# V2AI/EFG

Hardware: AMD Instinct MI355X
Metric: scenes/sec ConQueR 1-frame Waymo train step (higher is better)
Workload: dtype f32; 1 GPU; ConQueR res18 p3, 1-sweep Waymo-shaped scenes, 180000 pts/scene, 0.1 m voxels, 2 scenes/GPU, 900 queries, fwd+bwd+AdamW+OneCycle, graph of `value`: FPN levels / heads the reference evaluates and never reads are skipped (same losses and gradients; the line's `full_graph` object times the full reference graph); global_batch=2, parallelism=dp1

## Files before the change

### efg_amd/_lib.py

```python
import ctypes
import os

import torch

_LIB_PATH = os.path.join(os.path.dirname(os.path.abspath(__file__)), "lib", "libefg_hip.so")
_lib = None

c_void_p, c_int, c_int64, c_size_t, c_float = (ctypes.c_void_p, ctypes.c_int, ctypes.c_int64, ctypes.c_size_t,
                                               ctypes.c_float)

_SIGS = {
    "efg_last_error": (ctypes.c_char_p, []),
    "efg_version": (ctypes.c_char_p, []),
    "efg_capture_stream_create": (ctypes.c_int, [ctypes.POINTER(ctypes.c_void_p)]),
    "efg_capture_stream_destroy": (ctypes.c_int, [ctypes.c_void_p]),
    "efg_dynamic_voxelize_f32": (c_int, [c_void_p, c_int64, c_int, c_void_p, c_void_p, c_void_p, c_void_p]),
    "efg_hard_voxelize_workspace_bytes": (c_size_t, [c_int64, c_int, c_int, c_int, c_int, c_void_p, c_void_p]),
    "efg_hard_voxelize_f32": (c_int, [c_void_p, c_void_p, c_int, c_int, c_void_p, c_void_p, c_int, c_int, c_void_p,
                                      c_void_p, c_int, c_void_p, c_void_p, c_void_p, c_void_p, c_size_t, c_void_p]),
    "efg_hard_voxelize_debug_timeline": (c_size_t, [c_void_p]),
    "efg_scatter_workspace_bytes": (c_size_t, [c_int64, c_int, c_void_p]),
    "efg_scatter_index": (c_int, [c_void_p, c_int64, c_int, c_void_p, c_void_p, c_void_p, c_void_p, c_size_t,
                                  c_void_p]),
    "efg_scatter_reduce_workspace_bytes": (c_size_t, [c_int64, c_int]),
# ... 49 lines not shown
    "efg_box_attn_fused_backward_strided_f32": (c_int, [c_void_p] * 5 + [c_int, c_void_p, c_int, c_void_p, c_void_p] + [c_int] * 8 + [c_void_p] * 4 + [c_size_t, c_void_p]),
    "efg_box_attn_fused_backward_workspace_bytes": (c_size_t, [c_int] * 6),
    "efg_box_attn_fused_backward_f32": (c_int, [c_void_p] * 8 + [c_int] * 8 + [c_void_p] * 4 + [c_size_t, c_void_p]),
    "efg_boxes_bev_f32": (c_int, [c_void_p, c_int, c_void_p, c_int, c_int, c_void_p, c_void_p]),
    "efg_nms_workspace_bytes": (c_size_t, [c_int]),
    "efg_topk_unsorted_f32": (c_int, [c_void_p, c_int64, c_int, c_int, c_void_p, c_void_p, c_void_p]),
    "efg_box_refine_forward_f32": (c_int, [c_void_p, c_void_p, c_int64, c_float, c_void_p, c_void_p]),
    "efg_box_refine_backward_f32": (c_int, [c_void_p, c_void_p, c_void_p, c_int64, c_float, c_void_p, c_void_p, c_void_p]),
    "efg_add_layernorm_forward_f32": (c_int, [c_void_p] * 4 + [c_float, c_int64, c_int] + [c_void_p] * 5),
    "efg_add_layernorm_backward_workspace_bytes": (c_size_t, [c_int64, c_int]),
    "efg_add_layernorm_backward_f32": (c_int, [c_void_p] * 5 + [c_int64, c_int] + [c_void_p] * 4 + [c_size_t, c_void_p]),
    "efg_points_transform_filter_workspace_bytes": (c_size_t, [c_int64]),
    "efg_points_transform_filter_f32": (c_int, [c_void_p, c_int64, c_int, c_void_p, c_int, c_void_p, c_void_p, c_void_p,
                                                c_void_p, c_size_t, c_void_p]),
    "efg_points_gather_f32": (c_int, [c_void_p, c_void_p, c_int64, c_int, c_void_p, c_void_p]),
    "efg_match_cost_f32": (c_int, [c_void_p] * 4 + [c_int] * 5 + [c_float] * 6 + [c_void_p] * 3),
    "efg_focal_loss_forward_f32": (c_int, [c_void_p, c_void_p, c_int, c_int64, c_int, c_float, c_float, c_void_p, c_void_p,
                                           c_void_p]),
    "efg_focal_loss_backward_f32": (c_int, [c_void_p, c_void_p, c_int, c_int64, c_int, c_float, c_float, c_void_p,
                                            c_void_p, c_void_p, c_void_p]),
    "efg_box_loss_forward_f32": (c_int, [c_void_p] * 6 + [c_int64] + [c_int] * 4 + [c_void_p] * 4),
    "efg_box_loss_backward_f32": (c_int, [c_void_p] * 6 + [c_int64] + [c_int] * 4 + [c_void_p] * 5),
    "efg_rot_giou_paired_forward_f32": (c_int, [c_void_p, c_void_p, c_int64] + [c_void_p] * 4),
    "efg_rot_giou_paired_backward_f32": (c_int, [c_void_p, c_void_p, c_int64] + [c_void_p] * 5),
    "efg_bn_workspace_bytes": (c_size_t, [c_int]),
    "efg_bn_forward_f32": (c_int, [c_void_p] * 7 + [c_float, c_float, c_int64, c_int, c_int] + [c_void_p] * 4 +
                           [c_size_t, c_void_p]),
    "efg_bn_backward_f32": (c_int, [c_void_p] * 6 + [c_int64, c_int, c_int] + [c_void_p] * 5 + [c_size_t, c_void_p]),
    "efg_lsap_f32": (c_int, [c_void_p, c_int, c_int, c_int, c_void_p, c_void_p, c_void_p, c_void_p]),
    "efg_nms_f32": (c_int, [c_void_p, c_int, c_float, c_int, c_void_p, c_void_p, c_void_p, c_size_t, c_void_p]),
    "efg_spconv_tile_shape": (c_int, [c_int, c_int, c_int, c_int64, c_int64, c_void_p, c_void_p, c_void_p]),
    "efg_cylinder_select_f32": (c_int, [c_void_p, c_int64, c_int, c_int, c_float, c_void_p, c_void_p, c_int64, c_void_p,
                                        c_void_p, c_void_p, c_int, c_void_p, c_void_p]),
    "efg_attention_fwd_f32": (c_int, [c_void_p, c_int64, c_int64, c_void_p, c_void_p, c_int64, c_int64, c_int64, c_int, c_int,
                                      c_int, c_float, c_void_p, c_void_p, c_void_p]),
    "efg_attention_bwd_f32": (c_int, [c_void_p, c_int64, c_int64, c_void_p, c_void_p, c_int64, c_int64, c_void_p, c_void_p,
                                      c_void_p, c_int64, c_int, c_int, c_int, c_float, c_void_p, c_void_p, c_void_p,
                                      c_void_p]),
    "efg_attention_long_fwd_f32": (c_int, [c_void_p, c_int64, c_int64] * 3 + [c_void_p, c_int, c_int64, c_int, c_int, c_float,
                                                                             c_void_p, c_void_p, c_void_p]),
    "efg_attention_long_bwd_f32": (c_int, [c_void_p, c_int64, c_int64] * 3 + [c_void_p, c_int, c_void_p, c_void_p, c_void_p,
                                                                             c_int64, c_int, c_int, c_float, c_void_p, c_void_p,
                                                                             c_void_p, c_void_p, c_void_p]),
    "efg_relu_bwd_colsum_f32": (c_int, [c_void_p, c_void_p, c_int64, c_int, c_void_p, c_void_p, c_void_p, c_size_t, c_void_p]),
    "efg_nms_segmented_f32": (c_int, [c_void_p, c_void_p, c_int, c_float, c_int, c_void_p, c_void_p, c_void_p, c_size_t,
                                      c_void_p]),
    "efg_gn_workspace_bytes": (c_size_t, [c_int, c_int]),
    "efg_gn_forward_f32": (c_int, [c_void_p] * 3 + [c_float, c_int, c_int64, c_int, c_int] + [c_void_p] * 4 +
                           [c_size_t, c_void_p]),
    "efg_gn_backward_f32": (c_int, [c_void_p] * 5 + [c_int, c_int64, c_int, c_int] + [c_void_p] * 4 +
                            [c_size_t, c_void_p]),
    "efg_colsum_workspace_bytes": (c_size_t, [c_int64, c_int]),
    "efg_colsum_f32": (c_int, [c_void_p, c_int64, c_int, c_int64, c_void_p, c_void_p, c_size_t, c_void_p]),
    "efg_det_eval_max_pred": (c_int, []),
    "efg_det_eval_max_gt": (c_int, []),
    "efg_det_eval_pair_weights_f32": (c_int, [c_void_p] * 7 + [c_int] * 3 + [c_float] * 3 + [c_void_p, c_void_p]),
    "efg_det_eval_assign_f32": (c_int, [c_void_p] * 5 + [c_int] * 3 + [c_void_p] * 7),
    "efg_det_eval_accumulate": (c_int, [c_void_p, c_void_p, c_void_p, c_int] + [c_void_p] * 3),
    "efg_track_eval_mot_f32": (c_int, [c_void_p] * 6 + [c_int] * 4 + [c_void_p] * 5 + [c_int, c_void_p, c_int] +
                               [c_void_p] * 3),
    "efg_track_eval_accumulate": (c_int, [c_void_p, c_void_p, c_void_p, c_int, c_int] + [c_void_p] * 3),
    "efg_nusc_eval_max_gt": (c_int, []),
    "efg_nusc_eval_match_f32": (c_int, [c_void_p] * 3 + [c_int, c_int, c_int64, c_int64] + [c_float] * 4 +
                                [c_void_p, c_void_p]),
    "efg_nusc_eval_errors_f32": (c_int, [c_void_p] * 6 + [c_int64, c_int64, c_int] + [c_void_p] * 3),
    "efg_center_decode_max_cells": (c_int, []),
    "efg_center_decode_max_tasks": (c_int, []),
    "efg_center_decode_candidates_f32": (c_int, [c_void_p, c_void_p] + [c_int] * 4 + [c_float] * 6 + [c_void_p] * 6),
    "efg_circle_nms_f32": (c_int, [c_void_p] * 3 + [c_int, c_int, c_void_p, c_int, c_int] + [c_void_p] * 3),
    "efg_center_decode_boxes_f32": (c_int, [c_void_p, c_void_p] + [c_int] * 5 + [c_void_p] * 10),
    "efg_pillar_workspace_bytes": (c_size_t, []),
    "efg_pillar_forward_f32": (c_int, [c_void_p] * 9 + [c_float, c_float, c_int64] + [c_int] * 4 + [c_float] * 4 + [c_int] +
                               [c_void_p] * 5 + [c_size_t, c_int, c_void_p]),
    "efg_pillar_backward_f32": (c_int, [c_void_p] * 10 + [c_int64] + [c_int] * 4 + [c_float] * 4 + [c_int] + [c_void_p] * 4 +
                                [c_size_t, c_int, c_void_p]),
    "efg_pillar_scatter_f32": (c_int, [c_void_p, c_void_p, c_int64] + [c_int] * 4 + [c_void_p, c_void_p]),
    "efg_pillar_gather_f32": (c_int, [c_void_p, c_void_p, c_int64] + [c_int] * 4 + [c_void_p, c_void_p]),
}

_GEMM_SPLIT_SIGS = {
    "_pack_bytes": (c_size_t, [c_int, c_int]),
    "_pack_f32": (c_int, [c_void_p, c_int64, c_int64, c_int, c_int, c_void_p, c_void_p]),
    "_pack_linear_f32": (c_int, [c_void_p, c_int, c_int, c_void_p, c_void_p, c_void_p]),
    "_f32": (c_int, [c_void_p, c_int64, c_int, c_int64, c_void_p, c_int, c_void_p, c_int, c_void_p, c_int64, c_void_p]),
    "_wgrad_workspace_bytes": (c_size_t, [c_int64, c_int, c_int]),
    "_wgrad_f32": (c_int, [c_void_p, c_int64, c_void_p, c_int64, c_int64, c_int, c_int, c_void_p, c_void_p, c_size_t,
                           c_void_p]),
}
for _prefix in ("efg_gemm_bf16x3", "efg_gemm_bf16x6"):
    _SIGS.update({_prefix + _name: _sig for _name, _sig in _GEMM_SPLIT_SIGS.items()})

EXPORTED_SYMBOLS = tuple(_SIGS)


def lib_path():
    return _LIB_PATH


def _warn_if_stale():
    csrc = os.path.join(os.path.dirname(os.path.abspath(__file__)), "csrc")
    try:
        built = os.path.getmtime(_LIB_PATH)
        newer = [f for f in os.listdir(csrc) if os.path.getmtime(os.path.join(csrc, f)) > built + 1.0]
    except OSError:
        return
    if newer:
# ... 68 lines not shown
```

### efg_amd/build.py

```python
import os
import subprocess
import sys

_PKG = os.path.dirname(os.path.abspath(__file__))
_ROOT = os.path.dirname(_PKG)
CSRC = os.path.join(_PKG, "csrc")
LIB_DIR = os.path.join(_PKG, "lib")
LIB_PATH = os.path.join(LIB_DIR, "libefg_hip.so")

SOURCES = ["lib.cpp", "voxelize.hip", "voxelize_bins.hip", "voxelize_hash.hip", "scatter.hip", "spconv_index.hip", "spconv_conv.hip", "spconv_tiles.hip", "spconv_wgt.hip", "msda.hip", "box_fused.hip", "iou3d_nms.hip", "matcher.hip", "layernorm.hip", "augment.hip", "det_loss.hip", "rot_giou.hip", "batchnorm.hip", "colsum.hip", "crop.hip", "attention.hip", "gemm_bf16x3.hip", "gemm_bf16x6.hip", "topk.hip", "det_eval.hip", "track_eval.hip", "nusc_eval.hip", "center_decode.hip", "pillars.hip"]
FLAGS = ["--offload-arch=gfx950", "-O3", "-std=c++17", "-fPIC", "-munsafe-fp-atomics", "-ffp-contract=off",
         "-Wall", "-Wno-unused-function", "-I" + os.path.join(_ROOT, "include"), "-I" + CSRC]


def _stale(target, deps):
    if not os.path.exists(target):
        return True
    t = os.path.getmtime(target)
    return any(os.path.getmtime(d) > t for d in deps)


def build(force=False, verbose=False):
    os.makedirs(LIB_DIR, exist_ok=True)
    hipcc = os.environ.get("HIPCC", "/opt/rocm/bin/hipcc")
    headers = [os.path.join(CSRC, h) for h in os.listdir(CSRC) if h.endswith(".h")]
    headers.append(os.path.join(_ROOT, "include", "efg_hip.h"))
    objs = []
    procs = []
    for src in SOURCES:
        path = os.path.join(CSRC, src)
        if not os.path.exists(path):
            continue
        obj = os.path.join(LIB_DIR, os.path.splitext(src)[0] + ".o")
        objs.append(obj)
        if force or _stale(obj, [path] + headers):
            cmd = [hipcc] + FLAGS + ["-x", "hip", "-c", path, "-o", obj]
            if verbose:
                print(" ".join(cmd))
            procs.append((src, subprocess.Popen(cmd, stdout=subprocess.PIPE, stderr=subprocess.STDOUT)))
    for src, p in procs:
        out, _ = p.communicate()
        if p.returncode != 0:
            raise RuntimeError("hipcc failed on %s:\n%s" % (src, out.decode()))
        if verbose and out:
            print(out.decode())
    if force or procs or _stale(LIB_PATH, objs):
        cmd = [hipcc, "--offload-arch=gfx950", "-shared", "-fPIC", "-o", LIB_PATH] + objs
        subprocess.check_call(cmd)
    return LIB_PATH


if __name__ == "__main__":
    print(build(force="--force" in sys.argv, verbose=True))
```

### efg_amd/detection3d/utils.py

```python
import copy

import torch
import torch.nn.functional as F
from torch import nn

from ..operators.linear import Linear, linear


class MLP(nn.Module):

    def __init__(self, input_dim, hidden_dim, output_dim, num_layers):
        super().__init__()
        self.num_layers = num_layers
        h = [hidden_dim] * (num_layers - 1)
        self.layers = nn.ModuleList(Linear(n, k) for n, k in zip([input_dim] + h, h + [output_dim]))

    def forward(self, x):
        for i, layer in enumerate(self.layers):
            x = linear(x, layer.weight, layer.bias, relu=True) if i < self.num_layers - 1 else layer(x)
        return x


def get_clones(module, n):
    return nn.ModuleList([copy.deepcopy(module) for _ in range(n)])


def inverse_sigmoid(x, eps=1e-5):
    x = x.clamp(min=0, max=1)
    return torch.log(x.clamp(min=eps) / (1 - x).clamp(min=eps))


def box_cxcyczlwh_to_xyxyxy(x):
    c, s = x[..., :3], x[..., 3:6]
    return torch.cat((c - 0.5 * s, c + 0.5 * s), dim=-1)


def generalized_box3d_iou(boxes1, boxes2):
    boxes1 = torch.nan_to_num(boxes1)
    boxes2 = torch.nan_to_num(boxes2)
    vol1 = (boxes1[:, 3] - boxes1[:, 0]) * (boxes1[:, 4] - boxes1[:, 1]) * (boxes1[:, 5] - boxes1[:, 2])
    vol2 = (boxes2[:, 3] - boxes2[:, 0]) * (boxes2[:, 4] - boxes2[:, 1]) * (boxes2[:, 5] - boxes2[:, 2])
    lo = torch.max(boxes1[:, None, :3], boxes2[:, :3])
    hi = torch.min(boxes1[:, None, 3:], boxes2[:, 3:])
    lwh = (hi - lo).clamp(min=0)
    inter = lwh[:, :, 0] * lwh[:, :, 1] * lwh[:, :, 2]
    union = vol1[:, None] + vol2 - inter
    iou = inter / union
    lo = torch.min(boxes1[:, None, :3], boxes2[:, :3])
    hi = torch.max(boxes1[:, None, 3:], boxes2[:, 3:])
    whl = (hi - lo).clamp(min=0)
    vol = whl[:, :, 0] * whl[:, :, 1] * whl[:, :, 2]
    return iou - (vol - union) / vol


def pairwise_box3d_giou(boxes1, boxes2):
    boxes1 = torch.nan_to_num(boxes1)[..., :, None, :]
    boxes2 = torch.nan_to_num(boxes2)[..., None, :, :]
    vol1 = (boxes1[..., 3] - boxes1[..., 0]) * (boxes1[..., 4] - boxes1[..., 1]) * (boxes1[..., 5] - boxes1[..., 2])
    vol2 = (boxes2[..., 3] - boxes2[..., 0]) * (boxes2[..., 4] - boxes2[..., 1]) * (boxes2[..., 5] - boxes2[..., 2])
    lwh = (torch.min(boxes1[..., 3:], boxes2[..., 3:]) - torch.max(boxes1[..., :3], boxes2[..., :3])).clamp(min=0)
    inter = lwh[..., 0] * lwh[..., 1] * lwh[..., 2]
    union = vol1 + vol2 - inter
    whl = (torch.max(boxes1[..., 3:], boxes2[..., 3:]) - torch.min(boxes1[..., :3], boxes2[..., :3])).clamp(min=0)
    vol = whl[..., 0] * whl[..., 1] * whl[..., 2]
    return inter / union - (vol - union) / vol


def paired_box3d_giou(boxes1, boxes2):
    boxes1 = torch.nan_to_num(boxes1)
    boxes2 = torch.nan_to_num(boxes2)
    vol1 = (boxes1[:, 3] - boxes1[:, 0]) * (boxes1[:, 4] - boxes1[:, 1]) * (boxes1[:, 5] - boxes1[:, 2])
    vol2 = (boxes2[:, 3] - boxes2[:, 0]) * (boxes2[:, 4] - boxes2[:, 1]) * (boxes2[:, 5] - boxes2[:, 2])
# ... 119 lines not shown
```

### efg_amd/operators/linear.py

```python
import importlib
import os

import torch
import torch.nn.functional as F
from torch import nn
from torch.autograd import Function
from torch.autograd.function import once_differentiable

from .. import _lib as L


def column_sum(x2, out=None):
    L.require_gpu(x2)
    if x2.stride(1) != 1:
        x2 = x2.contiguous()
    rows, cols = x2.shape
    if out is None:
        out = torch.empty(cols, dtype=torch.float32, device=x2.device)
    ws_bytes = L.lib().efg_colsum_workspace_bytes(rows, cols)
    ws = torch.empty(max(ws_bytes, 16), dtype=torch.uint8, device=x2.device)
    L.check(L.lib().efg_colsum_f32(x2.data_ptr(), rows, cols, x2.stride(0) if rows > 1 else cols, L.ptr(out), L.ptr(ws),
                                   ws_bytes, L.stream()))
    return out

# ... 54 lines not shown
    if k >= _SPLIT_MIN_ROWS and k % _SPLITS == 0 and x2.is_contiguous() and g2.is_contiguous():
        gs = g2.view(_SPLITS, k // _SPLITS, g2.shape[1])
        xs = x2.view(_SPLITS, k // _SPLITS, x2.shape[1])
        return torch.bmm(gs.transpose(1, 2), xs).sum(0)
    if _WGRAD_ROWMAJOR:
        return g2.t().mm(x2)
    return x2.t().mm(g2).t()


class LinearFunction(Function):
    @staticmethod
    def forward(ctx, x, weight, bias, relu=False):
        x2 = x.reshape(-1, x.shape[-1])
        ctx.packed_dgrad = None
        G = _arm_gemm(x2)
        if G is not None:
            packed_fwd, ctx.packed_dgrad = G.pack_linear_both(weight.detach())
            y = G.gemm(x2, packed_fwd, weight.shape[0], bias=bias, relu=relu)
        elif relu and bias is not None and x2.shape[0] >= _FUSED_MIN_ROWS:
            y = torch._addmm_activation(bias, x2, weight.t(), use_gelu=False)
        else:
            y = torch.addmm(bias, x2, weight.t()) if bias is not None else x2.mm(weight.t())
            if relu:
                y = torch.relu_(y)
        ctx.relu = relu
        ctx.save_for_backward(x2, weight, y if relu else None)
        ctx.x_shape = x.shape
        return y.view(*x.shape[:-1], weight.shape[0])

    @staticmethod
    @once_differentiable
    def backward(ctx, grad):
        x2, weight, y = ctx.saved_tensors
        g2 = grad.reshape(-1, grad.shape[-1])
        gb = None
        if ctx.relu:
            if (ctx.needs_input_grad[2] and g2.is_contiguous() and y.is_contiguous() and g2.shape[1] % 4 == 0
                    and g2.data_ptr() % 16 == 0 and y.data_ptr() % 16 == 0):
                g2, gb = relu_backward_column_sum(g2, y)
            else:
                g2 = torch.ops.aten.threshold_backward(g2, y, 0)
        G = _arm_gemm(g2) if ctx.needs_input_grad[0] else None
        if G is not None:
            packed = ctx.packed_dgrad if ctx.packed_dgrad is not None else G.pack_linear(weight.detach(), True)
            gx = G.gemm(g2, packed, weight.shape[1]).view(ctx.x_shape)
        else:
            gx = g2.mm(weight).view(ctx.x_shape) if ctx.needs_input_grad[0] else None
        gw = weight_grad(x2, g2) if ctx.needs_input_grad[1] else None
        if gb is None and ctx.needs_input_grad[2]:
            gb = column_sum(g2)
        return gx, gw, gb, None


class SelfAttentionInProjFunction(Function):

    @staticmethod
    def forward(ctx, qk_in, v_in, weight, bias):
        c = weight.shape[1]
        q2, v2 = qk_in.reshape(-1, c), v_in.reshape(-1, c)
        qk = torch.addmm(bias[:2 * c], q2, weight[:2 * c].t())
        v = torch.addmm(bias[2 * c:], v2, weight[2 * c:].t())
        ctx.save_for_backward(q2, v2, weight)
        ctx.shapes = (qk_in.shape, v_in.shape)
        return qk.view(*qk_in.shape[:-1], 2 * c), v.view(*v_in.shape[:-1], c)

    @staticmethod
    @once_differentiable
    def backward(ctx, gqk, gv):
        q2, v2, weight = ctx.saved_tensors
        c = weight.shape[1]
        gqk2, gv2 = gqk.reshape(-1, 2 * c), gv.reshape(-1, c)
        if not gqk2.is_contiguous():
            gqk2 = gqk2.contiguous()
        if not gv2.is_contiguous():
            gv2 = gv2.contiguous()
        g_qk_in = gqk2.mm(weight[:2 * c]).view(ctx.shapes[0]) if ctx.needs_input_grad[0] else None
        g_v_in = gv2.mm(weight[2 * c:]).view(ctx.shapes[1]) if ctx.needs_input_grad[1] else None
        gw = gb = None
        if ctx.needs_input_grad[2]:
            gw = torch.empty_like(weight)
            torch.mm(gqk2.t(), q2, out=gw[:2 * c])
            torch.mm(gv2.t(), v2, out=gw[2 * c:])
        if ctx.needs_input_grad[3]:
            gb = torch.empty(3 * c, dtype=torch.float32, device=weight.device)
            column_sum(gqk2, out=gb[:2 * c])
            column_sum(gv2, out=gb[2 * c:])
        return g_qk_in, g_v_in, gw, gb


def self_attention_in_proj(qk_in, v_in, weight, bias):
    c = weight.shape[1]
    if (_SMALL_FUSED and qk_in.is_cuda and qk_in.dtype == torch.float32 and torch.is_grad_enabled() and bias is not None
            and (weight.requires_grad or qk_in.requires_grad or v_in.requires_grad)
            and os.environ.get("EFG_FUSED_LINEAR", "1") != "0"):
        return SelfAttentionInProjFunction.apply(qk_in, v_in, weight, bias)
    return F.linear(qk_in, weight[:2 * c], bias[:2 * c]), F.linear(v_in, weight[2 * c:], bias[2 * c:])


def linear(x, weight, bias=None, relu=False):
    if (x.is_cuda and x.dtype == torch.float32 and torch.is_grad_enabled()
            and (x.numel() >= _FUSED_MIN_ROWS * x.shape[-1] or (_SMALL_FUSED and relu and bias is not None and weight.shape[0] % 4 == 0))
            and (weight.requires_grad or (bias is not None and bias.requires_grad))
            and os.environ.get("EFG_FUSED_LINEAR", "1") != "0"):
        return LinearFunction.apply(x, weight, bias, relu)
    y = F.linear(x, weight, bias)
    return F.relu(y) if relu else y


class Linear(nn.Linear):
    def forward(self, x):
        return linear(x, self.weight, self.bias)
```

### include/efg_hip.h

```cpp
#ifndef EFG_HIP_H
#define EFG_HIP_H
#include <stddef.h>
#include <stdint.h>

#ifdef __cplusplus
extern "C" {
#endif

#define EFG_OK 0
#define EFG_E_INVALID (-1)
#define EFG_E_WORKSPACE (-2)
#define EFG_E_HIP (-3)

const char* efg_last_error(void);
const char* efg_version(void);

int efg_capture_stream_create(void** stream_out);
int efg_capture_stream_destroy(void* stream);


int efg_dynamic_voxelize_f32(const float* points, int64_t n, int f, const float* voxel_size_host,
                             const float* coors_range_host, int32_t* coors, void* stream);

size_t efg_hard_voxelize_workspace_bytes(int64_t n_total, int batch, int f, int max_points, int max_voxels,
// ... 167 lines not shown
                                    const float* range_host, float* out, int32_t* count, void* ws, size_t ws_bytes,
                                    void* stream);
int efg_points_gather_f32(const float* points, const int64_t* index, int64_t m, int f, float* out, void* stream);

int efg_match_cost_f32(const float* logits, const float* boxes, const int64_t* tgt_labels, const float* tgt_boxes,
                       int p, int b, int q, int c, int g, float w_class, float w_bbox, float w_giou, float w_rad,
                       float alpha, float gamma, const float* frame, float* cost, void* stream);
int efg_focal_loss_forward_f32(const float* logits, const int32_t* target_class, int layers, int64_t n, int c,
                               float alpha, float gamma, const float* denom, float* out, void* stream);
int efg_focal_loss_backward_f32(const float* logits, const int32_t* target_class, int layers, int64_t n, int c,
                                float alpha, float gamma, const float* denom, const float* grad_out,
                                float* grad_logits, void* stream);
int efg_box_loss_forward_f32(const float* boxes, const float* tgt_boxes, const int64_t* l_idx, const int64_t* b_idx,
                             const int64_t* q_idx, const int64_t* g_idx, int64_t n, int layers, int b, int q, int g,
                             const float* denom, const float* frame, float* out, void* stream);
int efg_box_loss_backward_f32(const float* boxes, const float* tgt_boxes, const int64_t* l_idx, const int64_t* b_idx,
                              const int64_t* q_idx, const int64_t* g_idx, int64_t n, int layers, int b, int q, int g,
                              const float* denom, const float* grad_out, const float* frame, float* grad_boxes,
                              void* stream);

int efg_rot_giou_paired_forward_f32(const float* a, const float* b, int64_t n, const float* frame, float* giou, float* iou,
                                    void* stream);
int efg_rot_giou_paired_backward_f32(const float* a, const float* b, int64_t n, const float* frame, const float* grad_giou,
                                     float* grad_a, float* grad_b, void* stream);

int efg_topk_unsorted_f32(const float* x, int64_t rows, int n, int k, float* values, int64_t* indices, void* stream);

int efg_box_refine_forward_f32(const float* delta, const float* anchor, int64_t n, float eps, float* out, void* stream);
int efg_box_refine_backward_f32(const float* grad, const float* out, const float* anchor, int64_t n, float eps,
                                float* grad_delta, float* grad_anchor, void* stream);

size_t efg_bn_workspace_bytes(int c);
int efg_bn_forward_f32(const float* x, const float* residual, const float* weight, const float* bias,
                       float* running_mean, float* running_var, int64_t* num_batches_tracked, float momentum, float eps,
                       int64_t m, int c, int relu, float* y, float* mean, float* invstd, void* ws, size_t ws_bytes,
                       void* stream);
int efg_bn_backward_f32(const float* dy, const float* x, const float* y, const float* weight, const float* mean,
                        const float* invstd, int64_t m, int c, int relu, float* dx, float* dresidual, float* dweight,
                        float* dbias, void* ws, size_t ws_bytes, void* stream);

size_t efg_gn_workspace_bytes(int batch, int c);
int efg_gn_forward_f32(const float* x, const float* weight, const float* bias, float eps, int batch, int64_t rows,
                       int c, int groups, float* y, float* mean, float* rstd, void* ws, size_t ws_bytes, void* stream);
int efg_gn_backward_f32(const float* dy, const float* x, const float* weight, const float* mean, const float* rstd,
                        int batch, int64_t rows, int c, int groups, float* dx, float* dweight, float* dbias, void* ws,
                        size_t ws_bytes, void* stream);

size_t efg_colsum_workspace_bytes(int64_t rows, int cols);
int efg_colsum_f32(const float* x, int64_t rows, int cols, int64_t row_stride, float* out, void* ws, size_t ws_bytes,
                   void* stream);
int efg_relu_bwd_colsum_f32(const float* g, const float* y, int64_t rows, int cols, float* g_out, float* out, void* ws,
                            size_t ws_bytes, void* stream);

size_t efg_gemm_bf16x3_pack_bytes(int k, int n);
int efg_gemm_bf16x3_pack_f32(const float* w, int64_t stride_k, int64_t stride_n, int k, int n, void* packed,
                             void* stream);
int efg_gemm_bf16x3_pack_linear_f32(const float* w, int n_out, int n_in, void* packed_fwd, void* packed_dgrad, void* stream);
int efg_gemm_bf16x3_f32(const float* a, int64_t m, int k, int64_t lda, const void* packed_b, int n, const float* bias,
                        int relu, float* c, int64_t ldc, void* stream);
size_t efg_gemm_bf16x3_wgrad_workspace_bytes(int64_t m, int n, int k);
int efg_gemm_bf16x3_wgrad_f32(const float* g, int64_t ldg, const float* x, int64_t ldx, int64_t m, int n, int k, float* dw,
                              void* ws, size_t ws_bytes, void* stream);

size_t efg_gemm_bf16x6_pack_bytes(int k, int n);
int efg_gemm_bf16x6_pack_f32(const float* w, int64_t stride_k, int64_t stride_n, int k, int n, void* packed,
                             void* stream);
int efg_gemm_bf16x6_pack_linear_f32(const float* w, int n_out, int n_in, void* packed_fwd, void* packed_dgrad, void* stream);
int efg_gemm_bf16x6_f32(const float* a, int64_t m, int k, int64_t lda, const void* packed_b, int n, const float* bias,
                        int relu, float* c, int64_t ldc, void* stream);
size_t efg_gemm_bf16x6_wgrad_workspace_bytes(int64_t m, int n, int k);
int efg_gemm_bf16x6_wgrad_f32(const float* g, int64_t ldg, const float* x, int64_t ldx, int64_t m, int n, int k, float* dw,
                              void* ws, size_t ws_bytes, void* stream);

int efg_det_eval_max_pred(void);
int efg_det_eval_max_gt(void);
int efg_det_eval_pair_weights_f32(const float* pred_boxes, const int32_t* pred_labels, const int32_t* pred_off,
                                  const float* gt_boxes, const int32_t* gt_labels, const int32_t* gt_off,
                                  const int64_t* blk_off, int n_frames, int max_pred, int max_gt, float thr_vehicle,
                                  float thr_pedestrian, float thr_cyclist, float* weights, void* stream);
int efg_det_eval_assign_f32(const float* weights, const int64_t* blk_off, const int32_t* pred_off, const int32_t* gt_off,
                            const int32_t* problems, int n_problems, int max_pred, int max_gt, const float* scores,
                            const float* pred_boxes, const float* gt_boxes, const int32_t* gt_level, int32_t* counts,
                            double* sums, void* stream);
int efg_det_eval_accumulate(const int32_t* counts, const double* sums, const int32_t* problems, int n_problems,
                            int64_t* total_counts, double* total_sums, void* stream);

int efg_track_eval_mot_f32(const float* weights, const int64_t* blk_off, const int32_t* trk_off, const int32_t* gt_off,
                           const int32_t* ranges, const int32_t* problems, int n_problems, int n_frames, int max_tracks,
                           int max_gt, const float* scores, const int32_t* track_ids, const int32_t* gt_ids,
                           const int32_t* gt_level, const float* cutoffs, int n_cutoffs, int32_t* last, int capacity,
                           int32_t* counts, double* sums, void* stream);
int efg_track_eval_accumulate(const int32_t* counts, const double* sums, const int32_t* problems, int n_problems,
                              int n_cutoffs, int64_t* total_counts, double* total_sums, void* stream);

int efg_nusc_eval_max_gt(void);
int efg_nusc_eval_match_f32(const float* pred_boxes, const float* gt_boxes, const int32_t* problems, int n_problems,
                            int max_gt, int64_t n_pred, int64_t n_gt, float thr0, float thr1, float thr2, float thr3,
                            int32_t* match, void* stream);
int efg_nusc_eval_errors_f32(const float* pred_boxes, const int32_t* pred_attr, const int32_t* pred_class,
                             const float* gt_boxes, const int32_t* gt_attr, const int32_t* match, int64_t n_pred,
                             int64_t n_gt, int barrier_class, int32_t* tp_bits, double* err, void* stream);

int efg_center_decode_max_cells(void);
int efg_center_decode_max_tasks(void);
int efg_center_decode_candidates_f32(const void* const* maps, const int32_t* num_classes, int n_tasks, int batch, int h,
                                     int w, float out_size_factor, float voxel_x, float voxel_y, float range_x,
// ... 31 lines not shown
```

Before: 64.07 scenes/s.

## Add fused narrow-linear HIP kernels for tiny in/out feature linears

Adds dedicated HIP kernels for linears where the output width or the input width is at most 16. They cover forward, and backward with fused dx, dw and db via per-block double partials plus a final reduction. The autograd linear path routes to these kernels when the shape qualifies and the heuristic judges them better, for example small-output regression heads or small-row cases. This replaces several generic GEMM and reduction launches with fewer fused ones, at the cost of new code paths and different summation order.

```diff
diff --git a/efg_amd/_lib.py b/efg_amd/_lib.py
--- a/efg_amd/_lib.py
+++ b/efg_amd/_lib.py
@@ -125,6 +125,14 @@
                             [c_size_t, c_void_p]),
     "efg_colsum_workspace_bytes": (c_size_t, [c_int64, c_int]),
     "efg_colsum_f32": (c_int, [c_void_p, c_int64, c_int, c_int64, c_void_p, c_void_p, c_size_t, c_void_p]),
+    "efg_linear_narrow_workspace_bytes": (c_size_t, [c_int64, c_int, c_int]),
+    "efg_linear_narrow_out_fwd_f32": (c_int, [c_void_p, c_int64, c_int64, c_void_p, c_void_p, c_int, c_int, c_void_p, c_void_p]),
+    "efg_linear_narrow_out_bwd_f32": (c_int, [c_void_p, c_int64, c_void_p, c_void_p, c_int64, c_int, c_int] + [c_void_p] * 4 +
+                                      [c_size_t, c_void_p]),
+    "efg_linear_narrow_in_fwd_f32": (c_int, [c_void_p, c_int64, c_int64, c_void_p, c_void_p, c_int, c_int, c_int, c_void_p,
+                                             c_void_p]),
+    "efg_linear_narrow_in_bwd_f32": (c_int, [c_void_p, c_int64, c_void_p, c_void_p, c_void_p, c_int64, c_int, c_int] +
+                                     [c_void_p] * 4 + [c_size_t, c_void_p]),
     "efg_det_eval_max_pred": (c_int, []),
     "efg_det_eval_max_gt": (c_int, []),
     "efg_det_eval_pair_weights_f32": (c_int, [c_void_p] * 7 + [c_int] * 3 + [c_float] * 3 + [c_void_p, c_void_p]),
diff --git a/efg_amd/build.py b/efg_amd/build.py
--- a/efg_amd/build.py
+++ b/efg_amd/build.py
@@ -8,7 +8,7 @@
 LIB_DIR = os.path.join(_PKG, "lib")
 LIB_PATH = os.path.join(LIB_DIR, "libefg_hip.so")
 
-SOURCES = ["lib.cpp", "voxelize.hip", "voxelize_bins.hip", "voxelize_hash.hip", "scatter.hip", "spconv_index.hip", "spconv_conv.hip", "spconv_tiles.hip", "spconv_wgt.hip", "msda.hip", "box_fused.hip", "iou3d_nms.hip", "matcher.hip", "layernorm.hip", "augment.hip", "det_loss.hip", "rot_giou.hip", "batchnorm.hip", "colsum.hip", "crop.hip", "attention.hip", "gemm_bf16x3.hip", "gemm_bf16x6.hip", "topk.hip", "det_eval.hip", "track_eval.hip", "nusc_eval.hip", "center_decode.hip", "pillars.hip"]
+SOURCES = ["lib.cpp", "voxelize.hip", "voxelize_bins.hip", "voxelize_hash.hip", "scatter.hip", "spconv_index.hip", "spconv_conv.hip", "spconv_tiles.hip", "spconv_wgt.hip", "msda.hip", "box_fused.hip", "iou3d_nms.hip", "matcher.hip", "layernorm.hip", "augment.hip", "det_loss.hip", "rot_giou.hip", "batchnorm.hip", "colsum.hip", "linear_narrow.hip", "crop.hip", "attention.hip", "gemm_bf16x3.hip", "gemm_bf16x6.hip", "topk.hip", "det_eval.hip", "track_eval.hip", "nusc_eval.hip", "center_decode.hip", "pillars.hip"]
 FLAGS = ["--offload-arch=gfx950", "-O3", "-std=c++17", "-fPIC", "-munsafe-fp-atomics", "-ffp-contract=off",
          "-Wall", "-Wno-unused-function", "-I" + os.path.join(_ROOT, "include"), "-I" + CSRC]
 
diff --git a/efg_amd/csrc/linear_narrow.hip b/efg_amd/csrc/linear_narrow.hip
--- /dev/null
+++ b/efg_amd/csrc/linear_narrow.hip
@@ -0,0 +1,543 @@
+#include "common.h"
+
+#include <algorithm>
+
+namespace efg {
+namespace {
+
+constexpr int kThreads = 256;
+constexpr int kMaxPartials = 512;
+constexpr int kMinRowsPerBlock = 32;
+constexpr int kMaxGrid = 2048;
+
+int log2_ceil(int v) {
+  int lg = 0;
+  while ((1 << lg) < v) ++lg;
+  return lg;
+}
+
+struct BwdPlan {
+  int rows_per_block, nblocks, pstride;
+};
+
+BwdPlan bwd_plan(int64_t rows, int in, int out) {
+  BwdPlan p;
+  p.rows_per_block = (int)std::max<int64_t>(kMinRowsPerBlock, ceil_div(std::max<int64_t>(rows, 1), kMaxPartials));
+  p.nblocks = (int)std::max<int64_t>(1, ceil_div(std::max<int64_t>(rows, 1), p.rows_per_block));
+  p.pstride = (int)align_up((size_t)out * in + out, 2);
+  return p;
+}
+
+__device__ __forceinline__ float4 ld4(const float* p) { return *reinterpret_cast<const float4*>(p); }
+__device__ __forceinline__ void st4(float* p, const float4& v) { *reinterpret_cast<float4*>(p) = v; }
+
+constexpr int kSumChunk = 40;
+
+template <int A>
+__device__ __forceinline__ void block_group_sum(double (&a)[A], int lg, double* __restrict__ sm) {
+  constexpr int CH = A < kSumChunk ? A : kSumChunk;
+  const int lane = threadIdx.x & 63, wave = threadIdx.x >> 6;
+  for (int m = 1 << lg; m < 64; m <<= 1) {
+#pragma unroll
+    for (int i = 0; i < A; ++i) a[i] += __shfl_xor(a[i], m, 64);
+  }
+  const int w0 = lg <= 6 ? 1 : 1 << (lg - 6);
+#pragma unroll
+  for (int c0 = 0; c0 < A; c0 += CH) {
+    if (c0) __syncthreads();
+    if (wave >= w0) {
+#pragma unroll
+      for (int i = 0; i < CH; ++i)
+        if (c0 + i < A) sm[((wave - w0) * CH + i) * 64 + lane] = a[c0 + i];
+    }
+    __syncthreads();
+    if (wave < w0) {
+      for (int o = wave + w0; o < kThreads / 64; o += w0) {
+#pragma unroll
+        for (int i = 0; i < CH; ++i)
+          if (c0 + i < A) a[c0 + i] += sm[((o - w0) * CH + i) * 64 + lane];
+      }
+    }
+  }
+}
+
+
+template <int V, int S>
+__device__ __forceinline__ void scatter_step(float (&v)[V], int lg, int lane, int& first, bool& owner) {
+  if (S >= lg) return;
+  constexpr int n = V >> (S + 1), m = 1 << S;
+  const bool hi = (lane & m) != 0;
+  if constexpr (n >= 1) {
+#pragma unroll
+    for (int i = 0; i < n; ++i) {
+      const float send = hi ? v[i] : v[i + n];
+      const float keep = hi ? v[i + n] : v[i];
+      v[i] = keep + __shfl_xor(send, m, 64);
+    }
+    if (hi) first += n;
+  } else {
+    v[0] += __shfl_xor(v[0], m, 64);
+    if (hi) owner = false;
+  }
+}
+
+template <int NT>
+__global__ void __launch_bounds__(kThreads)
+narrow_out_fwd_kernel(const float* __restrict__ x, long long rows, long long x_stride, const float* __restrict__ w,
+                      const float* __restrict__ bias, int K, int N, int lg, float* __restrict__ y) {
+  extern __shared__ float4 s_w[];
+  constexpr int R = 4;
+  const int S = K >> 2;
+  for (int i = threadIdx.x; i < NT * S; i += kThreads) {
+    const int n = i / S;
+    s_w[i] = n < N ? ld4(w + (long long)n * K + (long long)(i - n * S) * 4) : float4{0.f, 0.f, 0.f, 0.f};
+  }
+  __syncthreads();
+  const int lane = threadIdx.x & 63, wave = threadIdx.x >> 6;
+  const int L = 1 << lg, sub = lane & (L - 1), rsub = lane >> lg, rps = 64 >> lg;
+  const long long tile = (long long)(kThreads / 64) * R * rps;
+  for (long long base = (long long)blockIdx.x * tile; base < rows; base += (long long)gridDim.x * tile) {
+    long long r[R];
+    float acc[R * NT];
+#pragma unroll
+    for (int u = 0; u < R; ++u) r[u] = base + (long long)(u * (kThreads / 64) + wave) * rps + rsub;
+#pragma unroll
+    for (int i = 0; i < R * NT; ++i) acc[i] = 0.f;
+    for (int s = sub; s < S; s += L) {
+      float4 xv[R];
+#pragma unroll
+      for (int u = 0; u < R; ++u)
+        xv[u] = r[u] < rows ? ld4(x + r[u] * x_stride + (long long)s * 4) : float4{0.f, 0.f, 0.f, 0.f};
+#pragma unroll
+      for (int n = 0; n < NT; ++n) {
+        const float4 wv = s_w[n * S + s];
+#pragma unroll
+        for (int u = 0; u < R; ++u) {
+          float t = acc[u * NT + n];
+          t = fmaf(xv[u].x, wv.x, t);
+          t = fmaf(xv[u].y, wv.y, t);
+          t = fmaf(xv[u].z, wv.z, t);
+          t = fmaf(xv[u].w, wv.w, t);
+          acc[u * NT + n] = t;
+        }
+      }
+    }
+    int first = 0;
+    bool owner = true;
+    scatter_step<R * NT, 0>(acc, lg, lane, first, owner);
+    scatter_step<R * NT, 1>(acc, lg, lane, first, owner);
+    scatter_step<R * NT, 2>(acc, lg, lane, first, owner);
+    scatter_step<R * NT, 3>(acc, lg, lane, first, owner);
+    scatter_step<R * NT, 4>(acc, lg, lane, first, owner);
+    scatter_step<R * NT, 5>(acc, lg, lane, first, owner);
+    const int held = max((R * NT) >> lg, 1);
+    if (owner) {
+#pragma unroll
+      for (int i = 0; i < R * NT; ++i) {
+        const int idx = first + i, u = idx / NT, n = idx - u * NT;
+        const long long ru = base + (long long)(u * (kThreads / 64) + wave) * rps + rsub;
+        if (i < held && ru < rows && n < N) y[ru * N + n] = bias ? acc[i] + bias[n] : acc[i];
+      }
+    }
+  }
+}
+
+template <int NT, bool DX>
+__global__ void __launch_bounds__(kThreads)
+narrow_out_bwd_kernel(const float* __restrict__ x, long long x_stride, const float* __restrict__ dy,
+                      const float* __restrict__ w, long long rows, int K, int N, int lg, int rows_per_block,
+                      float* __restrict__ dx, double* __restrict__ partial, int pstride) {
+  constexpr int A = NT * 5;
+  constexpr int U = NT >= 16 ? 1 : NT == 1 ? 8 : 4;
+  __shared__ double sm[3 * (A < kSumChunk ? A : kSumChunk) * 64];
+  const int slot = threadIdx.x & ((1 << lg) - 1), group = threadIdx.x >> lg, G = kThreads >> lg;
+  const bool ok = slot < (K >> 2);
+  float4 wv[NT];
+  if constexpr (DX) {
+#pragma unroll
+    for (int n = 0; n < NT; ++n)
+      wv[n] = ok && n < N ? ld4(w + (long long)n * K + (long long)slot * 4) : float4{0.f, 0.f, 0.f, 0.f};
+  }
+  double a[A];
+#pragma unroll
+  for (int i = 0; i < A; ++i) a[i] = 0.0;
+  const long long r0 = (long long)blockIdx.x * rows_per_block;
+  const long long r1 = min(rows, r0 + rows_per_block);
+  for (long long base = r0; base < r1; base += (long long)G * U) {
+    float4 xv[U];
+    float g[U][NT];
+#pragma unroll
+    for (int u = 0; u < U; ++u) {
+      const long long r = base + (long long)u * G + group;
+      const bool valid = r < r1;
+      xv[u] = valid && ok ? ld4(x + r * x_stride + (long long)slot * 4) : float4{0.f, 0.f, 0.f, 0.f};
+#pragma unroll
+      for (int n = 0; n < NT; ++n) g[u][n] = valid && n < N ? dy[r * N + n] : 0.f;
+    }
+#pragma unroll
+    for (int u = 0; u < U; ++u) {
+#pragma unroll
+      for (int n = 0; n < NT; ++n) {
+        const double gn = (double)g[u][n];
+        a[n * 4 + 0] = fma(gn, (double)xv[u].x, a[n * 4 + 0]);
+        a[n * 4 + 1] = fma(gn, (double)xv[u].y, a[n * 4 + 1]);
+        a[n * 4 + 2] = fma(gn, (double)xv[u].z, a[n * 4 + 2]);
+        a[n * 4 + 3] = fma(gn, (double)xv[u].w, a[n * 4 + 3]);
+        a[NT * 4 + n] += gn;
+      }
+      if constexpr (DX) {
+        const long long r = base + (long long)u * G + group;
+        if (r < r1 && ok) {
+          float4 d{0.f, 0.f, 0.f, 0.f};
+#pragma unroll
+          for (int n = 0; n < NT; ++n) {
+            d.x = fmaf(g[u][n], wv[n].x, d.x);
+            d.y = fmaf(g[u][n], wv[n].y, d.y);
+            d.z = fmaf(g[u][n], wv[n].z, d.z);
+            d.w = fmaf(g[u][n], wv[n].w, d.w);
+          }
+          st4(dx + r * K + (long long)slot * 4, d);
+        }
+      }
+    }
+  }
+  block_group_sum<A>(a, lg, sm);
+  if (group == 0 && ok) {
+    double* p = partial + (long long)blockIdx.x * pstride;
+#pragma unroll
+    for (int n = 0; n < NT; ++n) {
+      if (n < N) {
+#pragma unroll
+        for (int j = 0; j < 4; ++j) p[(long long)n * K + (long long)slot * 4 + j] = a[n * 4 + j];
+        if (slot == 0) p[(long long)N * K + n] = a[NT * 4 + n];
+      }
+    }
+  }
+}
+
+
+template <int KT>
+__global__ void __launch_bounds__(kThreads)
+narrow_in_fwd_kernel(const float* __restrict__ x, long long rows, long long x_stride, const float* __restrict__ w,
+                     const float* __restrict__ bias, int K, int N, int lg, int relu, float* __restrict__ y) {
+  constexpr int U = 4;
+  const int slot = threadIdx.x & ((1 << lg) - 1), group = threadIdx.x >> lg, G = kThreads >> lg;
+  if (slot >= (N >> 2)) return;
+  float wv[4][KT];
+#pragma unroll
+  for (int j = 0; j < 4; ++j) {
+#pragma unroll
+    for (int k = 0; k < KT; ++k) wv[j][k] = k < K ? w[(long long)(slot * 4 + j) * K + k] : 0.f;
+  }
+  const float4 bv = bias ? ld4(bias + slot * 4) : float4{0.f, 0.f, 0.f, 0.f};
+  const long long tile = (long long)G * U;
+  for (long long base = (long long)blockIdx.x * tile; base < rows; base += (long long)gridDim.x * tile) {
+#pragma unroll
+    for (int u = 0; u < U; ++u) {
+      const long long r = base + (long long)u * G + group;
+      if (r >= rows) continue;
+      float o[4] = {0.f, 0.f, 0.f, 0.f};
+#pragma unroll
+      for (int k = 0; k < KT; ++k) {
+        const float xk = k < K ? x[r * x_stride + k] : 0.f;
+#pragma unroll
+        for (int j = 0; j < 4; ++j) o[j] = fmaf(xk, wv[j][k], o[j]);
+      }
+      if (bias) {
+        o[0] += bv.x;
+        o[1] += bv.y;
+        o[2] += bv.z;
+        o[3] += bv.w;
+      }
+      if (relu) {
+#pragma unroll
+        for (int j = 0; j < 4; ++j) o[j] = o[j] < 0.f ? 0.f : o[j];
+      }
+      st4(y + r * N + (long long)slot * 4, float4{o[0], o[1], o[2], o[3]});
+    }
+  }
+}
+
+template <int KT, bool DX>
+__global__ void __launch_bounds__(kThreads)
+narrow_in_bwd_kernel(const float* __restrict__ x, long long x_stride, const float* __restrict__ dy,
+                     const float* __restrict__ y, const float* __restrict__ w, long long rows, int K, int N, int lg,
+                     int rows_per_block, float* __restrict__ dx, double* __restrict__ partial, int pstride) {
+  constexpr int A = 4 * KT + 4;
+  constexpr int U = 2;
+  __shared__ double sm[3 * (A < kSumChunk ? A : kSumChunk) * 64];
+  __shared__ float s_dx[kThreads / 64][KT];
+  const int lane = threadIdx.x & 63, wave = threadIdx.x >> 6;
+  const int slot = threadIdx.x & ((1 << lg) - 1), group = threadIdx.x >> lg, G = kThreads >> lg;
+  const bool ok = slot < (N >> 2);
+  float wv[4][KT];
+  if constexpr (DX) {
+#pragma unroll
+    for (int j = 0; j < 4; ++j) {
+#pragma unroll
+      for (int k = 0; k < KT; ++k) wv[j][k] = ok && k < K ? w[(long long)(slot * 4 + j) * K + k] : 0.f;
+    }
+  }
+  double a[A];
+#pragma unroll
+  for (int i = 0; i < A; ++i) a[i] = 0.0;
+  const long long r0 = (long long)blockIdx.x * rows_per_block;
+  const long long r1 = min(rows, r0 + rows_per_block);
+  for (long long base = r0; base < r1; base += (long long)G * U) {
+#pragma unroll
+    for (int u = 0; u < U; ++u) {
+      const long long r = base + (long long)u * G + group;
+      const bool valid = r < r1;
+      float4 gv{0.f, 0.f, 0.f, 0.f};
+      if (valid && ok) {
+        gv = ld4(dy + r * N + (long long)slot * 4);
+        if (y) {
+          const float4 m = ld4(y + r * N + (long long)slot * 4);
+          gv.x = m.x > 0.f ? gv.x : 0.f;
+          gv.y = m.y > 0.f ? gv.y : 0.f;
+          gv.z = m.z > 0.f ? gv.z : 0.f;
+          gv.w = m.w > 0.f ? gv.w : 0.f;
+        }
+      }
+      const float g[4] = {gv.x, gv.y, gv.z, gv.w};
+#pragma unroll
+      for (int k = 0; k < KT; ++k) {
+        const double xk = valid && k < K ? (double)x[r * x_stride + k] : 0.0;
+#pragma unroll
+        for (int j = 0; j < 4; ++j) a[j * KT + k] = fma((double)g[j], xk, a[j * KT + k]);
+      }
+#pragma unroll
+      for (int j = 0; j < 4; ++j) a[4 * KT + j] += (double)g[j];
+      if constexpr (DX) {
+        float d[KT];
+#pragma unroll
+        for (int k = 0; k < KT; ++k) {
+          float t = 0.f;
+#pragma unroll
+          for (int j = 0; j < 4; ++j) t = fmaf(g[j], wv[j][k], t);
+          d[k] = t;
+        }
+        const int lw = lg < 6 ? lg : 6;
+        for (int m = 1; m < (1 << lw); m <<= 1) {
+#pragma unroll
+          for (int k = 0; k < KT; ++k) d[k] += __shfl_xor(d[k], m, 64);
+        }
+        if (lg <= 6) {
+          if (valid && (lane & ((1 << lw) - 1)) == 0) {
+#pragma unroll
+            for (int k = 0; k < KT; ++k)
+              if (k < K) dx[r * K + k] = d[k];
+          }
+        } else {
+          const int w0 = 1 << (lg - 6);
+          if (lane == 0) {
+#pragma unroll
+            for (int k = 0; k < KT; ++k) s_dx[wave][k] = d[k];
+          }
+          __syncthreads();
+          if (valid && (wave & (w0 - 1)) == 0 && lane < K) {
+            float t = s_dx[wave][lane];
+            for (int o = 1; o < w0; ++o) t += s_dx[wave + o][lane];
+            dx[r * K + lane] = t;
+          }
+          __syncthreads();
+        }
+      }
+    }
+  }
+  block_group_sum<A>(a, lg, sm);
+  if (group == 0 && ok) {
+    double* p = partial + (long long)blockIdx.x * pstride;
+#pragma unroll
+    for (int j = 0; j < 4; ++j) {
+#pragma unroll
+      for (int k = 0; k < KT; ++k)
+        if (k < K) p[(long long)(slot * 4 + j) * K + k] = a[j * KT + k];
+      p[(long long)N * K + slot * 4 + j] = a[4 * KT + j];
+    }
+  }
+}
+
+template <int kWaves>
+__global__ void __launch_bounds__(64 * kWaves)
+narrow_final_kernel(const double* __restrict__ partial, int nblocks, int pstride, int n_dw, int n_db,
+                    float* __restrict__ dw, float* __restrict__ db) {
+  __shared__ double sm[kWaves][64];
+  const int lane = threadIdx.x & 63, wave = threadIdx.x >> 6;
+  const int c = blockIdx.x * 64 + lane;
+  const bool ok = c < n_dw + n_db;
+  double s[4] = {0.0, 0.0, 0.0, 0.0};
+  if (ok) {
+    int b = wave;
+    for (; b + 3 * kWaves < nblocks; b += 4 * kWaves) {
+#pragma unroll
+      for (int i = 0; i < 4; ++i) s[i] += partial[(long long)(b + kWaves * i) * pstride + c];
+    }
+    for (; b < nblocks; b += kWaves) s[0] += partial[(long long)b * pstride + c];
+  }
+  sm[wave][lane] = (s[0] + s[1]) + (s[2] + s[3]);
+  __syncthreads();
+  if (wave == 0 && ok) {
+    double t = 0.0;
+#pragma unroll
+    for (int w = 0; w < kWaves; ++w) t += sm[w][lane];
+    if (c < n_dw)
+      dw[c] = (float)t;
+    else
+      db[c - n_dw] = (float)t;
+  }
+}
+
+int launch_final(const BwdPlan& p, const double* partial, int in, int out, float* dw, float* db, hipStream_t st) {
+  const int n_dw = in * out, n_db = db ? out : 0;
+  const dim3 grid((unsigned)ceil_div(n_dw + n_db, 64));
+  if (p.nblocks > 64)
+    hipLaunchKernelGGL(narrow_final_kernel<16>, grid, dim3(1024), 0, st, partial, p.nblocks, p.pstride, n_dw, n_db, dw, db);
+  else
+    hipLaunchKernelGGL(narrow_final_kernel<4>, grid, dim3(256), 0, st, partial, p.nblocks, p.pstride, n_dw, n_db, dw, db);
+  EFG_LAUNCH_CHECK();
+  return EFG_OK;
+}
+
+bool aligned16(const void* p) { return (reinterpret_cast<uintptr_t>(p) & 15) == 0; }
+
+int zero_reductions(int in, int out, float* dw, float* db, hipStream_t st) {
+  EFG_HIP_TRY(hipMemsetAsync(dw, 0, sizeof(float) * (size_t)in * out, st));
+  if (db) EFG_HIP_TRY(hipMemsetAsync(db, 0, sizeof(float) * out, st));
+  return EFG_OK;
+}
+
+int narrow_out_nt(int out) { return out <= 1 ? 1 : out <= 4 ? 4 : out <= 8 ? 8 : 16; }
+int narrow_in_kt(int in) { return in <= 4 ? 4 : 16; }
+
+}
+}
+
+using namespace efg;
+
+#define EFG_NARROW_OUT_SHAPE(name)                                                                                  \
+  EFG_CHECK_ARG(rows >= 0 && out >= 1 && out <= 16 && in >= 4 && in <= 1024 && in % 4 == 0,                         \
+                name ": unsupported shape %lld rows, %d -> %d (out <= 16, in %% 4 == 0, in <= 1024)", (long long)rows, in, out)
+#define EFG_NARROW_IN_SHAPE(name)                                                                                   \
+  EFG_CHECK_ARG(rows >= 0 && in >= 1 && in <= 16 && out >= 4 && out <= 1024 && out % 4 == 0,                        \
+                name ": unsupported shape %lld rows, %d -> %d (in <= 16, out %% 4 == 0, out <= 1024)", (long long)rows, in, out)
+
+extern "C" size_t efg_linear_narrow_workspace_bytes(int64_t rows, int in, int out) {
+  if (rows < 0 || in < 1 || out < 1 || in > 1024 || out > 1024) return 0;
+  const BwdPlan p = bwd_plan(rows, in, out);
+  return align_up(sizeof(double) * (size_t)p.pstride * (size_t)p.nblocks, 256);
+}
+
+extern "C" int efg_linear_narrow_out_fwd_f32(const float* x, int64_t rows, int64_t x_stride, const float* w,
+                                             const float* bias, int in, int out, float* y, void* stream) {
+  EFG_NARROW_OUT_SHAPE("linear_narrow_out_fwd");
+  if (rows == 0) return EFG_OK;
+  EFG_CHECK_ARG(x && w && y, "linear_narrow_out_fwd: null pointer");
+  EFG_CHECK_ARG(x_stride >= in && x_stride % 4 == 0 && aligned16(x) && aligned16(w),
+                "linear_narrow_out_fwd: x rows and w must be 16-byte aligned (row stride %lld)", (long long)x_stride);
+  hipStream_t st = (hipStream_t)stream;
+  const int lg = std::min(6, log2_ceil(in / 4));
+  const int64_t tile = 16ll * (64 >> lg);
+  const dim3 grid((unsigned)std::min<int64_t>(kMaxGrid, ceil_div(rows, tile)));
+  const int nt = narrow_out_nt(out);
+  const size_t lds = sizeof(float) * (size_t)nt * in;
+#define EFG_LAUNCH(NT)                                                                                             \
+  hipLaunchKernelGGL(narrow_out_fwd_kernel<NT>, grid, dim3(kThreads), lds, st, x, (long long)rows, (long long)x_stride, w, \
+                     bias, in, out, lg, y)
+  if (nt == 1) EFG_LAUNCH(1);
+  else if (nt == 4) EFG_LAUNCH(4);
+  else if (nt == 8) EFG_LAUNCH(8);
+  else EFG_LAUNCH(16);
+#undef EFG_LAUNCH
+  EFG_LAUNCH_CHECK();
+  return EFG_OK;
+}
+
+extern "C" int efg_linear_narrow_out_bwd_f32(const float* x, int64_t x_stride, const float* dy, const float* w,
+                                             int64_t rows, int in, int out, float* dx, float* dw, float* db, void* ws,
+                                             size_t ws_bytes, void* stream) {
+  EFG_NARROW_OUT_SHAPE("linear_narrow_out_bwd");
+  EFG_CHECK_ARG(dw, "linear_narrow_out_bwd: null weight gradient");
+  hipStream_t st = (hipStream_t)stream;
+  if (rows == 0) return zero_reductions(in, out, dw, db, st);
+  EFG_CHECK_ARG(x && dy && w && ws, "linear_narrow_out_bwd: null pointer");
+  EFG_CHECK_ARG(x_stride >= in && x_stride % 4 == 0 && aligned16(x) && aligned16(w) && aligned16(dx) && aligned16(ws),
+                "linear_narrow_out_bwd: x rows, w, dx and the workspace must be 16-byte aligned (row stride %lld)",
+                (long long)x_stride);
+  const BwdPlan p = bwd_plan(rows, in, out);
+  EFG_CHECK_ARG(ws_bytes >= sizeof(double) * (size_t)p.pstride * (size_t)p.nblocks, "linear_narrow_out_bwd: workspace too small");
+  const int lg = log2_ceil(in / 4);
+  double* partial = static_cast<double*>(ws);
+  const int nt = narrow_out_nt(out);
+#define EFG_LAUNCH(NT, DX)                                                                                          \
+  hipLaunchKernelGGL((narrow_out_bwd_kernel<NT, DX>), dim3(p.nblocks), dim3(kThreads), 0, st, x, (long long)x_stride, dy, w, \
+                     (long long)rows, in, out, lg, p.rows_per_block, dx, partial, p.pstride)
+#define EFG_LAUNCH_DX(NT) \
+  do {                    \
+    if (dx)               \
+      EFG_LAUNCH(NT, true);  \
+    else                  \
+      EFG_LAUNCH(NT, false); \
+  } while (0)
+  if (nt == 1) EFG_LAUNCH_DX(1);
+  else if (nt == 4) EFG_LAUNCH_DX(4);
+  else if (nt == 8) EFG_LAUNCH_DX(8);
+  else EFG_LAUNCH_DX(16);
+#undef EFG_LAUNCH_DX
+#undef EFG_LAUNCH
+  EFG_LAUNCH_CHECK();
+  return launch_final(p, partial, in, out, dw, db, st);
+}
+
+extern "C" int efg_linear_narrow_in_fwd_f32(const float* x, int64_t rows, int64_t x_stride, const float* w,
+                                            const float* bias, int in, int out, int relu, float* y, void* stream) {
+  EFG_NARROW_IN_SHAPE("linear_narrow_in_fwd");
+  if (rows == 0) return EFG_OK;
+  EFG_CHECK_ARG(x && w && y, "linear_narrow_in_fwd: null pointer");
+  EFG_CHECK_ARG(x_stride >= in && aligned16(bias) && aligned16(y),
+                "linear_narrow_in_fwd: bias and y must be 16-byte aligned, row stride %lld >= in", (long long)x_stride);
+  hipStream_t st = (hipStream_t)stream;
+  const int lg = log2_ceil(out / 4);
+  const int64_t tile = 4ll * (kThreads >> lg);
+  const dim3 grid((unsigned)std::min<int64_t>(kMaxGrid, ceil_div(rows, tile)));
+#define EFG_LAUNCH(KT)                                                                                             \
+  hipLaunchKernelGGL(narrow_in_fwd_kernel<KT>, grid, dim3(kThreads), 0, st, x, (long long)rows, (long long)x_stride, w, bias, \
+                     in, out, lg, relu, y)
+  if (narrow_in_kt(in) == 4) EFG_LAUNCH(4);
+  else EFG_LAUNCH(16);
+#undef EFG_LAUNCH
+  EFG_LAUNCH_CHECK();
+  return EFG_OK;
+}
+
+extern "C" int efg_linear_narrow_in_bwd_f32(const float* x, int64_t x_stride, const float* dy, const float* y,
+                                            const float* w, int64_t rows, int in, int out, float* dx, float* dw, float* db,
+                                            void* ws, size_t ws_bytes, void* stream) {
+  EFG_NARROW_IN_SHAPE("linear_narrow_in_bwd");
+  EFG_CHECK_ARG(dw, "linear_narrow_in_bwd: null weight gradient");
+  hipStream_t st = (hipStream_t)stream;
+  if (rows == 0) return zero_reductions(in, out, dw, db, st);
+  EFG_CHECK_ARG(x && dy && w && ws, "linear_narrow_in_bwd: null pointer");
+  EFG_CHECK_ARG(x_stride >= in && aligned16(dy) && aligned16(y),
+                "linear_narrow_in_bwd: dy and y must be 16-byte aligned, row stride %lld >= in", (long long)x_stride);
+  const BwdPlan p = bwd_plan(rows, in, out);
+  EFG_CHECK_ARG(ws_bytes >= sizeof(double) * (size_t)p.pstride * (size_t)p.nblocks, "linear_narrow_in_bwd: workspace too small");
+  const int lg = log2_ceil(out / 4);
+  double* partial = static_cast<double*>(ws);
+#define EFG_LAUNCH(KT, DX)                                                                                          \
+  hipLaunchKernelGGL((narrow_in_bwd_kernel<KT, DX>), dim3(p.nblocks), dim3(kThreads), 0, st, x, (long long)x_stride, dy, y, w, \
+                     (long long)rows, in, out, lg, p.rows_per_block, dx, partial, p.pstride)
+#define EFG_LAUNCH_DX(KT) \
+  do {                    \
+    if (dx)               \
+      EFG_LAUNCH(KT, true);  \
+    else                  \
+      EFG_LAUNCH(KT, false); \
+  } while (0)
+  if (narrow_in_kt(in) == 4) EFG_LAUNCH_DX(4);
+  else EFG_LAUNCH_DX(16);
+#undef EFG_LAUNCH_DX
+#undef EFG_LAUNCH
+  EFG_LAUNCH_CHECK();
+  return launch_final(p, partial, in, out, dw, db, st);
+}
diff --git a/efg_amd/detection3d/utils.py b/efg_amd/detection3d/utils.py
--- a/efg_amd/detection3d/utils.py
+++ b/efg_amd/detection3d/utils.py
@@ -17,7 +17,7 @@
 
     def forward(self, x):
         for i, layer in enumerate(self.layers):
-            x = linear(x, layer.weight, layer.bias, relu=True) if i < self.num_layers - 1 else layer(x)
+            x = linear(x, layer.weight, layer.bias, relu=i < self.num_layers - 1)
         return x
 
 
diff --git a/efg_amd/operators/linear.py b/efg_amd/operators/linear.py
--- a/efg_amd/operators/linear.py
+++ b/efg_amd/operators/linear.py
@@ -130,6 +130,90 @@
         return gx, gw, gb, None
 
 
+def narrow_kind(x, weight, bias, relu):
+    if os.environ.get("EFG_NARROW_LINEAR", "1") == "0" or os.environ.get("EFG_FUSED_LINEAR", "1") == "0":
+        return None
+    if not (x.is_cuda and x.dtype == torch.float32 and weight.dim() == 2 and x.dim() >= 1 and x.shape[-1] == weight.shape[1]):
+        return None
+    for p in (weight, bias):
+        if p is not None and not (p.is_cuda and p.dtype == torch.float32 and p.is_contiguous() and p.data_ptr() % 16 == 0):
+            return None
+    n, k = weight.shape
+    if n <= 16 and k % 4 == 0 and 4 <= k <= 1024 and not relu:
+        return "out"
+    if 1 <= k <= 16 and n % 4 == 0 and 4 <= n <= 1024:
+        return "in"
+    return None
+
+
+def narrow_wins(kind, x, weight):
+    rows = x.numel() // weight.shape[1]
+    if kind == "out":
+        return weight.shape[0] <= 4 or rows < _FUSED_MIN_ROWS
+    return rows < _FUSED_MIN_ROWS and not x.requires_grad
+
+
+def _narrow_rows(kind, t2):
+    if t2.stride(1) != 1 or (kind == "out" and (t2.data_ptr() % 16 != 0 or (t2.shape[0] > 1 and t2.stride(0) % 4 != 0))):
+        t2 = t2.clone(memory_format=torch.contiguous_format)
+    return t2
+
+
+def _row_stride(t2):
+    return t2.stride(0) if t2.shape[0] > 1 else t2.shape[1]
+
+
+def narrow_forward(kind, x2, weight, bias, relu):
+    rows, (n, k) = x2.shape[0], weight.shape
+    y = torch.empty(rows, n, dtype=torch.float32, device=x2.device)
+    if kind == "out":
+        L.check(L.lib().efg_linear_narrow_out_fwd_f32(x2.data_ptr(), rows, _row_stride(x2), L.ptr(weight), L.ptr(bias), k, n,
+                                                      L.ptr(y), L.stream()))
+    else:
+        L.check(L.lib().efg_linear_narrow_in_fwd_f32(x2.data_ptr(), rows, _row_stride(x2), L.ptr(weight), L.ptr(bias), k, n,
+                                                     int(relu), L.ptr(y), L.stream()))
+    return y
+
+
+def narrow_backward(kind, x2, g2, weight, y, want_dx, has_bias):
+    (n, k), rows, dev = weight.shape, x2.shape[0], x2.device
+    dx = torch.empty(rows, k, dtype=torch.float32, device=dev) if want_dx else None
+    dw = torch.empty_like(weight)
+    db = torch.empty(n, dtype=torch.float32, device=dev) if has_bias else None
+    ws_bytes = L.lib().efg_linear_narrow_workspace_bytes(rows, k, n)
+    ws = torch.empty(max(ws_bytes, 16), dtype=torch.uint8, device=dev)
+    if kind == "out":
+        L.check(L.lib().efg_linear_narrow_out_bwd_f32(x2.data_ptr(), _row_stride(x2), L.ptr(g2), L.ptr(weight), rows, k, n,
+                                                      L.ptr(dx), L.ptr(dw), L.ptr(db), L.ptr(ws), ws_bytes, L.stream()))
+    else:
+        L.check(L.lib().efg_linear_narrow_in_bwd_f32(x2.data_ptr(), _row_stride(x2), L.ptr(g2), L.ptr(y), L.ptr(weight), rows,
+                                                     k, n, L.ptr(dx), L.ptr(dw), L.ptr(db), L.ptr(ws), ws_bytes, L.stream()))
+    return dx, dw, db
+
+
+class NarrowLinearFunction(Function):
+
+    @staticmethod
+    def forward(ctx, x, weight, bias, relu, kind):
+        x2 = _narrow_rows(kind, x.reshape(-1, x.shape[-1]))
+        y = narrow_forward(kind, x2, weight, bias, relu)
+        ctx.kind, ctx.relu, ctx.has_bias, ctx.x_shape = kind, relu, bias is not None, x.shape
+        ctx.save_for_backward(x2, weight, y if relu else None)
+        return y.view(*x.shape[:-1], weight.shape[0])
+
+    @staticmethod
+    @once_differentiable
+    def backward(ctx, grad):
+        x2, weight, y = ctx.saved_tensors
+        n, k = weight.shape
+        g2 = grad.reshape(-1, n)
+        if not g2.is_contiguous() or g2.data_ptr() % 16 != 0:
+            g2 = g2.clone(memory_format=torch.contiguous_format)
+        dx, dw, db = narrow_backward(ctx.kind, x2, g2, weight, y, ctx.needs_input_grad[0], ctx.has_bias)
+        return (dx.view(ctx.x_shape) if dx is not None else None, dw if ctx.needs_input_grad[1] else None,
+                db if ctx.needs_input_grad[2] else None, None, None)
+
+
 class SelfAttentionInProjFunction(Function):
 
     @staticmethod
@@ -176,6 +260,10 @@
 
 
 def linear(x, weight, bias=None, relu=False):
+    if torch.is_grad_enabled() and (x.requires_grad or weight.requires_grad or (bias is not None and bias.requires_grad)):
+        kind = narrow_kind(x, weight, bias, relu)
+        if kind is not None and narrow_wins(kind, x, weight):
+            return NarrowLinearFunction.apply(x, weight, bias, relu, kind)
     if (x.is_cuda and x.dtype == torch.float32 and torch.is_grad_enabled()
             and (x.numel() >= _FUSED_MIN_ROWS * x.shape[-1] or (_SMALL_FUSED and relu and bias is not None and weight.shape[0] % 4 == 0))
             and (weight.requires_grad or (bias is not None and bias.requires_grad))
diff --git a/include/efg_hip.h b/include/efg_hip.h
--- a/include/efg_hip.h
+++ b/include/efg_hip.h
@@ -243,6 +243,17 @@
 int efg_relu_bwd_colsum_f32(const float* g, const float* y, int64_t rows, int cols, float* g_out, float* out, void* ws,
                             size_t ws_bytes, void* stream);
 
+size_t efg_linear_narrow_workspace_bytes(int64_t rows, int in, int out);
+int efg_linear_narrow_out_fwd_f32(const float* x, int64_t rows, int64_t x_stride, const float* w, const float* bias, int in,
+                                  int out, float* y, void* stream);
+int efg_linear_narrow_out_bwd_f32(const float* x, int64_t x_stride, const float* dy, const float* w, int64_t rows, int in,
+                                  int out, float* dx, float* dw, float* db, void* ws, size_t ws_bytes, void* stream);
+int efg_linear_narrow_in_fwd_f32(const float* x, int64_t rows, int64_t x_stride, const float* w, const float* bias, int in,
+                                 int out, int relu, float* y, void* stream);
+int efg_linear_narrow_in_bwd_f32(const float* x, int64_t x_stride, const float* dy, const float* y_mask, const float* w,
+                                 int64_t rows, int in, int out, float* dx, float* dw, float* db, void* ws, size_t ws_bytes,
+                                 void* stream);
+
 size_t efg_gemm_bf16x3_pack_bytes(int k, int n);
 int efg_gemm_bf16x3_pack_f32(const float* w, int64_t stride_k, int64_t stride_n, int k, int n, void* packed,
                              void* stream);
```

Measured after the change: 64.40 scenes/s, median of 3. About the same (+0.5%).
